# czbiohub-sf/yogo

Measured on AMD Instinct MI355X. Metric: training images/sec (772x1032 gray), higher is better.
Workload: dtype bf16; 1 GPU; BASELINE configs[2]: full train step (fwd+loss+bwd+clamp+AdamW), base_model, 772x1032x1 uint8, 7 classes; per_gpu_batch=128, global_batch=128, parallelism=dp1

## Files before the change

### yogo_amd/csrc/conv_first_fused_bwd.hip

```cpp
#include "common.h"
#include <mutex>
#include <type_traits>
#include <utility>

typedef unsigned int u32x4 __attribute__((ext_vector_type(4)));
typedef int i32x4 __attribute__((ext_vector_type(4)));
typedef float f32x4 __attribute__((ext_vector_type(4)));
typedef float f32x2 __attribute__((ext_vector_type(2)));
typedef __bf16 bf16x8 __attribute__((ext_vector_type(8)));

struct DgFirstParams {
  const u32x4* g;
  const u32x4* wp;
  const unsigned char* img;
  const unsigned short* signs;
  float* part;
  const u32x4* x;
  float* slab;
  float* bias_part;
  int B, H, W, Mpad, act, ncol;
  int tiles_per_row, tile_rows, seg, segs_per_img, nsegs;
  unsigned m_tpr, m_spi;
};

namespace {
constexpr int DF_NJ = 9, DF_PER = 2 * DF_NJ + 2, DF_COUT = 16;
__device__ __forceinline__ int df_udivm1(int n, int d, unsigned m) { return d == 1 ? n : (int)__umulhi((unsigned)n, m); }
__device__ __forceinline__ unsigned df_u(unsigned v) { return (unsigned)__builtin_amdgcn_readfirstlane((int)v); }
__device__ __forceinline__ i32x4 df_rsrc(const void* ptr, unsigned bytes) {
  const unsigned long long a = reinterpret_cast<unsigned long long>(ptr);
  return i32x4{(int)df_u((unsigned)a), (int)df_u((unsigned)(a >> 32) & 0xFFFFu), (int)df_u(bytes), 0x00020000};
}
__device__ __forceinline__ void df_dma16(i32x4 rs, unsigned lds_addr, int voff) {
  unsigned keep;
  lds_addr = df_u(lds_addr);
  asm volatile("s_mov_b32 %0, m0\n\ts_mov_b32 m0, %2\n\ts_nop 4\n\tbuffer_load_dwordx4 %1, %3, 0 offen lds\n\ts_mov_b32 m0, %0"
               : "=&s"(keep) : "v"(voff), "s"(lds_addr), "s"(rs) : "memory");
}
__device__ __forceinline__ void df_dma4(i32x4 rs, unsigned lds_addr, int voff) {
  unsigned keep;
  lds_addr = df_u(lds_addr);
  asm volatile("s_mov_b32 %0, m0\n\ts_mov_b32 m0, %2\n\ts_nop 4\n\tbuffer_load_dword %1, %3, 0 offen lds\n\ts_mov_b32 m0, %0"
               : "=&s"(keep) : "v"(voff), "s"(lds_addr), "s"(rs) : "memory");
}
__device__ __forceinline__ void df_wait_dma() { asm volatile("s_waitcnt vmcnt(0)" ::: "memory"); }
__device__ __forceinline__ bf16x8 df_tr8(const unsigned char* a, int second) {
  typedef __bf16 bf16x4 __attribute__((ext_vector_type(4)));
  typedef bf16x4 __attribute__((address_space(3))) * lds_v4;
  const bf16x4 lo = __builtin_amdgcn_ds_read_tr16_b64_v4bf16((lds_v4)(a));
  const bf16x4 hi = __builtin_amdgcn_ds_read_tr16_b64_v4bf16((lds_v4)(a + second));
  return __builtin_shufflevector(lo, hi, 0, 1, 2, 3, 4, 5, 6, 7);
}
}

#ifndef DF_WAVES_PER_EU
#define DF_WAVES_PER_EU 2
#endif
#ifndef DF_NPF
#define DF_NPF 6
#endif
#ifndef DF_NPF_WG
#define DF_NPF_WG 3
#endif
namespace {
template <class F, int... I>
__device__ __forceinline__ void df_static_for(F&& f, std::integer_sequence<int, I...>) {
  (f(std::integral_constant<int, I>{}), ...);
}
}
template <int R, int NWV, bool WG>
__global__ __launch_bounds__(64 * NWV) __attribute__((amdgpu_waves_per_eu(DF_WAVES_PER_EU))) void conv_bf16_dgrad_first_bwd_kernel(const DgFirstParams p) {
  extern __shared__ __attribute__((aligned(16))) u32x4 lds_u[];
  constexpr int OOB = (int)0x80000000u;
  constexpr int KB = 4, NR = R + 2, ROWU = 34, TU = KB * NR * ROWU, NDMA = (TU + 63) / 64;
  constexpr int IR = 2 * R + 1, IROWB = 72, IDW = IROWB / 4, IU = IR * IDW, NIDMA = (IU + 63) / 64;
  constexpr int SU = R * 16, NSDMA = (SU + 63) / 64;
  static_assert(!WG || (R % 2) == 0, "a piece of the staged x tile is two whole rows");
  constexpr int NXDMA = WG ? R : 0;
  constexpr int WAVE_BYTES = NDMA * 1024 + NIDMA * 256 + NSDMA * 256 + NXDMA * 1024;
  constexpr int CONST_BYTES = ((IR * IROWB + 15) / 16) * 16;
  const int tid = threadIdx.x, lane = tid & 63, c16 = lane & 15, g4 = lane >> 4;
  const int wave = __builtin_amdgcn_readfirstlane(tid >> 6);
  const int H = p.H, W = p.W, IH0 = 2 * H, IW0 = 2 * W;
  const int kcb = H * W * 16;
  const bool leaky = p.act == ACT_LEAKY;
  const unsigned my_addr = (unsigned)(wave * WAVE_BYTES), my_img_addr = my_addr + NDMA * 1024, my_sg_addr = my_img_addr + NIDMA * 256;
  [[maybe_unused]] const unsigned my_x_addr = my_sg_addr + NSDMA * 256;
  const unsigned ones_addr = (unsigned)(NWV * WAVE_BYTES), zeros_addr = ones_addr + CONST_BYTES;
  const u32x4* my_tile = lds_u + wave * (WAVE_BYTES / 16);
  const unsigned char* lds8 = reinterpret_cast<const unsigned char*>(lds_u);
  {
    unsigned* cw = reinterpret_cast<unsigned*>(lds_u) + ones_addr / 4;
    for (int e = tid; e < CONST_BYTES / 4; e += 64 * NWV) {
      cw[e] = 0x01010101u;
      cw[e + CONST_BYTES / 4] = 0u;
    }
  }
  __syncthreads();

  bf16x8 wv[9];
#pragma unroll
  for (int tp = 0; tp < 9; ++tp) wv[tp] = __builtin_bit_cast(bf16x8, p.wp[(tp * KB + g4) * p.Mpad + c16]);

  int rel[NDMA];
  unsigned rc[NDMA];
#pragma unroll
  for (int i = 0; i < NDMA; ++i) {
    const int u = i * 64 + lane;
    const int kb = u / (NR * ROWU), rem = u - kb * (NR * ROWU);
    const int r = rem / ROWU, cc = rem - r * ROWU;
    rel[i] = u < TU ? kb * kcb + (r * W + cc) * 16 : OOB;
    rc[i] = u < TU ? (unsigned)(r << 16 | cc) : 0xFFFFFFFFu;
  }
  unsigned irc[NIDMA];
#pragma unroll
  for (int i = 0; i < NIDMA; ++i) {
    const int e = i * 64 + lane;
    const int r = e / IDW, d = e - r * IDW;
    irc[i] = e < IU ? (unsigned)(r << 16 | d) : 0xFFFFFFFFu;
  }
  const int xj = c16 < 9 ? c16 : 0, kh = xj / 3, kw = xj - 3 * kh;
  const unsigned x_addr = c16 < 9 ? my_img_addr + (unsigned)(kh * IROWB + ((3 + 8 * g4 + kw) & ~3)) : (c16 == 9 ? ones_addr : zeros_addr) + (unsigned)(8 * g4);
  const unsigned x_sh = c16 < 9 ? (unsigned)((3 + kw) & 3) : 0u;
  const unsigned sg_addr = my_sg_addr + (unsigned)(8 * g4);
  const unsigned sg_pos = (unsigned)(c16 < 4 ? c16 : c16 < 8 ? c16 + 4 : c16 < 12 ? c16 - 4 : c16);

  f32x4 d2p = {0.f, 0.f, 0.f, 0.f}, d2n = {0.f, 0.f, 0.f, 0.f};
  f32x4 wacc[WG ? 2 : 1][WG ? 9 : 1], bacc[WG ? 2 : 1];
#pragma unroll
  for (int c = 0; c < (WG ? 2 : 1); ++c) {
    bacc[c] = f32x4{0.f, 0.f, 0.f, 0.f};
#pragma unroll
    for (int t = 0; t < (WG ? 9 : 1); ++t) wacc[c][t] = f32x4{0.f, 0.f, 0.f, 0.f};
  }
  [[maybe_unused]] const unsigned tr_g = my_addr + (unsigned)((((c16 & 3) >> 1) * NR * ROWU + 8 * g4 + (c16 >> 2)) * 16 + (c16 & 1) * 8);
  [[maybe_unused]] const unsigned tr_x = my_x_addr + (unsigned)((((c16 & 3) >> 1) * R * 32 + 8 * g4 + (c16 >> 2)) * 16 + (c16 & 1) * 8);
  const u32x4 ones_op = {0x3F803F80u, 0x3F803F80u, 0x3F803F80u, 0x3F803F80u};

  const int xcd = blockIdx.x & 7, slot = blockIdx.x >> 3, nslot = gridDim.x >> 3;
  const int s8 = (p.nsegs + 7) >> 3, s_end = min(p.nsegs, (xcd + 1) * s8);
  for (int sgm = xcd * s8 + slot * NWV + wave; sgm < s_end; sgm += nslot * NWV) {
    const int b = df_udivm1(sgm, p.segs_per_img, p.m_spi);
    const int t = sgm - b * p.segs_per_img;
    const int sy = df_udivm1(t, p.tiles_per_row, p.m_tpr), ox0 = (t - sy * p.tiles_per_row) * 32;
    const int ty_end = min(p.tile_rows, (sy + 1) * p.seg);
   for (int ty = sy * p.seg; ty < ty_end; ++ty) {
    const int oy0 = ty * R;
    {
      const i32x4 rs_g = df_rsrc(p.g + (size_t)b * KB * H * W, (unsigned)(KB * kcb));
      const int iy0 = oy0 - 1, ix0 = ox0 - 1;
      const int base = (iy0 * W + ix0) * 16;
      if (iy0 >= 0 && iy0 + NR <= H && ix0 >= 0 && ix0 + ROWU <= W) {
#pragma unroll
        for (int i = 0; i < NDMA; ++i) df_dma16(rs_g, my_addr + (unsigned)i * 1024u, (i + 1) * 64 <= TU ? rel[i] + base : (rel[i] == OOB ? OOB : rel[i] + base));
      } else {
#pragma unroll
        for (int i = 0; i < NDMA; ++i) {
          const int r = (int)(rc[i] >> 16), c = (int)(rc[i] & 0xFFFFu);
          const bool ok = ((unsigned)(iy0 + r) < (unsigned)H) && ((unsigned)(ix0 + c) < (unsigned)W);
          df_dma16(rs_g, my_addr + (unsigned)i * 1024u, ok ? rel[i] + base : OOB);
        }
      }
      const i32x4 rs_i = df_rsrc(p.img + (size_t)b * IH0 * IW0, (unsigned)(IH0 * IW0));
      const int jy0 = 2 * oy0 - 1, jx0 = 2 * ox0 - 4;
#pragma unroll
      for (int i = 0; i < NIDMA; ++i) {
        const int r = (int)(irc[i] >> 16), d = (int)(irc[i] & 0xFFFFu);
        const int iy = jy0 + r, ix = jx0 + 4 * d;
        const bool ok = ((unsigned)iy < (unsigned)IH0) && ((unsigned)ix < (unsigned)IW0);
        df_dma4(rs_i, my_img_addr + (unsigned)i * 256u, ok ? iy * IW0 + ix : OOB);
      }
      if (leaky) {
        const i32x4 rs_s = df_rsrc(p.signs + (size_t)b * H * W, (unsigned)(H * W * 2));
#pragma unroll
        for (int i = 0; i < NSDMA; ++i) {
          const int e = i * 64 + lane, r = e >> 4, d = e & 15;
          const bool ok = e < SU && oy0 + r < H && ox0 + 2 * d < W;
          df_dma4(rs_s, my_sg_addr + (unsigned)i * 256u, ok ? ((oy0 + r) * W + ox0 + 2 * d) * 2 : OOB);
        }
      }
      if constexpr (WG) {
        const i32x4 rs_x = df_rsrc(p.x + (size_t)b * 2 * H * W, (unsigned)(2 * kcb));
        const int hi = lane >> 5, col = lane & 31;
        const int xo = ((oy0 + hi) * W + ox0 + col) * 16;
        const bool cok = ox0 + col < W;
#pragma unroll
        for (int i = 0; i < NXDMA; ++i) {
          constexpr int dummy = 0; (void)dummy;
          const int kb = (2 * i) / R, row0 = (2 * i) % R;
          df_dma16(rs_x, my_x_addr + (unsigned)i * 1024u, (cok && oy0 + row0 + hi < H) ? xo + kb * kcb + row0 * W * 16 : OOB);
        }
      }
    }
    const bool right = ox0 + 32 > W;
    df_wait_dma();
    const u32x4* bt = my_tile + g4 * NR * ROWU + c16;
#pragma unroll
    for (int rr = 0; rr < R; ++rr) {
      if (oy0 + rr >= H) break;
      constexpr int NST = WG ? 36 : 18, NPF = WG ? DF_NPF_WG : DF_NPF;
      f32x4 acc[2];
      bf16x8 ring[NPF];
      [[maybe_unused]] bf16x8 xt;
      auto load = [&](auto s_tag) {
        constexpr int S = decltype(s_tag)::value;
        if constexpr (S < 18) {
          constexpr int pb = S / 9, tp = S % 9, ky = tp / 3, kx = tp % 3;
          ring[S % NPF] = __builtin_bit_cast(bf16x8, bt[(rr + ky) * ROWU + 16 * pb + kx]);
        } else {
          constexpr int cbk = (S - 18) / 9, tp = (S - 18) % 9, ky = tp / 3, kx = tp % 3;
          ring[S % NPF] = df_tr8(lds8 + tr_g + ((cbk * 2 * NR + rr + 2 - ky) * ROWU + 2 - kx) * 16, 64);
        }
      };
      auto use = [&](auto s_tag) {
        constexpr int S = decltype(s_tag)::value;
        if constexpr (S < 18) {
          constexpr int pb = S / 9, tp = S % 9;
          acc[pb] = __builtin_amdgcn_mfma_f32_16x16x32_bf16(ring[S % NPF], wv[tp], tp == 0 ? f32x4{0.f, 0.f, 0.f, 0.f} : acc[pb], 0, 0, 0);
        } else if constexpr (WG) {
          constexpr int cbk = (S - 18) / 9, tp = (S - 18) % 9;
          wacc[cbk][tp] = __builtin_amdgcn_mfma_f32_16x16x32_bf16(ring[S % NPF], xt, wacc[cbk][tp], 0, 0, 0);
          if constexpr (tp == 4) bacc[cbk] = __builtin_amdgcn_mfma_f32_16x16x32_bf16(ring[S % NPF], __builtin_bit_cast(bf16x8, ones_op), bacc[cbk], 0, 0, 0);
        }
      };
      unsigned xr[2][3];
      unsigned sw[2][2] = {{0xFFFFFFFFu, 0xFFFFFFFFu}, {0xFFFFFFFFu, 0xFFFFFFFFu}};
      u32x4 xop, gpos, gneg;
      auto p3 = [&](auto k_tag) {
        constexpr int K = decltype(k_tag)::value;
        typedef __bf16 bf16x2 __attribute__((ext_vector_type(2)));
        if constexpr (K == 0) {
#pragma unroll
          for (int pb = 0; pb < 2; ++pb) {
            const unsigned char* xa = lds8 + x_addr + rr * (2 * IROWB) + 32 * pb;
            xr[pb][0] = *reinterpret_cast<const unsigned*>(xa);
            xr[pb][1] = *reinterpret_cast<const unsigned*>(xa + 4);
            xr[pb][2] = *reinterpret_cast<const unsigned*>(xa + 8);
            if (leaky) {
              const unsigned long long s2 = *reinterpret_cast<const unsigned long long*>(lds8 + sg_addr + rr * 64 + 32 * pb);
              sw[pb][0] = (unsigned)s2;
              sw[pb][1] = (unsigned)(s2 >> 32);
            }
          }
        } else if constexpr (K == 1 || K == 2) {
          constexpr int pb = K - 1;
          const unsigned lo4 = __builtin_amdgcn_alignbyte(xr[pb][1], xr[pb][0], x_sh), hi4 = __builtin_amdgcn_alignbyte(xr[pb][2], xr[pb][1], x_sh);
          const unsigned xs = __builtin_amdgcn_perm(hi4, lo4, 0x06040200u);
          const bf16x2 q0 = {(__bf16)(float)(xs & 0xFFu), (__bf16)(float)((xs >> 8) & 0xFFu)};
          const bf16x2 q1 = {(__bf16)(float)((xs >> 16) & 0xFFu), (__bf16)(float)(xs >> 24)};
          xop[2 * pb] = __builtin_bit_cast(unsigned, q0);
          xop[2 * pb + 1] = __builtin_bit_cast(unsigned, q1);
        } else if constexpr (K == 3 || K == 4) {
          constexpr int pb = K - 3;
#pragma unroll
          for (int q = 0; q < 2; ++q) {
            const bf16x2 dq = {(__bf16)acc[pb][2 * q], (__bf16)acc[pb][2 * q + 1]};
            unsigned dw = __builtin_bit_cast(unsigned, dq);
            if (right && ox0 + 16 * pb + 4 * g4 + 2 * q >= W) dw = 0u;
            const unsigned m = leaky ? __umul24((sw[pb][q] >> sg_pos) & 0x00010001u, 0xFFFFu) : 0xFFFFFFFFu;
            const unsigned pos = dw & m;
            gpos[2 * pb + q] = pos;
            gneg[2 * pb + q] = dw ^ pos;
          }
        } else if constexpr (K == 5) {
          d2p = __builtin_amdgcn_mfma_f32_16x16x32_bf16(__builtin_bit_cast(bf16x8, xop), __builtin_bit_cast(bf16x8, gpos), d2p, 0, 0, 0);
        } else {
          d2n = __builtin_amdgcn_mfma_f32_16x16x32_bf16(__builtin_bit_cast(bf16x8, xop), __builtin_bit_cast(bf16x8, gneg), d2n, 0, 0, 0);
        }
      };
      df_static_for([&](auto s_tag) { load(s_tag); }, std::make_integer_sequence<int, NPF>{});
      __builtin_amdgcn_sched_barrier(0);
      df_static_for(
          [&](auto s_tag) {
            constexpr int S = decltype(s_tag)::value;
            use(s_tag);
            if constexpr (S + NPF < NST) load(std::integral_constant<int, S + NPF>{});
            if constexpr (WG) {
              if constexpr (S == 10) xt = df_tr8(lds8 + tr_x + rr * 512, 64);
              if constexpr (S == 18) p3(std::integral_constant<int, 0>{});
              if constexpr (S == 23) p3(std::integral_constant<int, 1>{});
              if constexpr (S == 25) p3(std::integral_constant<int, 2>{});
              if constexpr (S == 27) p3(std::integral_constant<int, 3>{});
              if constexpr (S == 29) p3(std::integral_constant<int, 4>{});
              if constexpr (S == 31) p3(std::integral_constant<int, 5>{});
              if constexpr (S == 32) p3(std::integral_constant<int, 6>{});
            } else {
              if constexpr (S == 12) p3(std::integral_constant<int, 0>{});
              if constexpr (S == 15) p3(std::integral_constant<int, 1>{});
              if constexpr (S == 16) p3(std::integral_constant<int, 2>{});
            }
            __builtin_amdgcn_sched_barrier(0);
          },
          std::make_integer_sequence<int, NST>{});
      if constexpr (!WG) {
        p3(std::integral_constant<int, 3>{});
        p3(std::integral_constant<int, 4>{});
        p3(std::integral_constant<int, 5>{});
        p3(std::integral_constant<int, 6>{});
      }
    }
   }
  }
  float* prow = p.part + (size_t)(blockIdx.x * NWV + wave) * p.ncol;
#pragma unroll
  for (int i = 0; i < 4; ++i) {
    const int j = 4 * g4 + i;
    const float v = d2p[i] + LEAKY_SLOPE * d2n[i];
    if (j < DF_NJ) prow[c16 * DF_PER + j] = v;
    else if (j == DF_NJ) prow[c16 * DF_PER + 2 * DF_NJ] = v;
  }
  if (g4 == 0) prow[c16 * DF_PER + 2 * DF_NJ + 1] = 0.f;
  for (int e = lane; e < DF_COUT * DF_NJ; e += 64) prow[(e / DF_NJ) * DF_PER + DF_NJ + e % DF_NJ] = 0.f;
  for (int e = lane; e < DF_NJ + DF_NJ * DF_NJ; e += 64) prow[DF_COUT * DF_PER + e] = 0.f;
  if constexpr (WG) {
    constexpr int NE = 9 * 32 * 16, STRIDE = NE + 32;
    static_assert(NWV * STRIDE * 4 <= NWV * WAVE_BYTES + 2 * CONST_BYTES, "the reduction uses the kernel's LDS allocation");
    __syncthreads();
    float* red = reinterpret_cast<float*>(lds_u) + wave * STRIDE;
#pragma unroll
    for (int cbk = 0; cbk < 2; ++cbk)
#pragma unroll
      for (int i = 0; i < 4; ++i) {
        const int co = 16 * cbk + 4 * g4 + i;
#pragma unroll
        for (int tp = 0; tp < 9; ++tp) red[(tp * 32 + co) * 16 + c16] = wacc[cbk][tp][i];
        if (c16 == 0) red[NE + co] = bacc[cbk][i];
      }
    __syncthreads();
    const float* r0 = reinterpret_cast<const float*>(lds_u);
    float* sl = p.slab + (size_t)blockIdx.x * NE;
    float* bp = p.bias_part + (size_t)blockIdx.x * 32;
    for (int e = tid; e < STRIDE; e += 64 * NWV) {
      float v = r0[e];
#pragma unroll
      for (int w = 1; w < NWV; ++w) v += r0[w * STRIDE + e];
      if (e < NE) sl[e] = v;
      else bp[e - NE] = v;
    }
  }
}

#ifndef DF_TILE_ROWS
#define DF_TILE_ROWS 6
#endif
#ifndef DF_TILE_ROWS_WG
#define DF_TILE_ROWS_WG 4
#endif
#ifndef DF_WAVES
#define DF_WAVES 4
#endif
namespace {
constexpr int DF_NWV = DF_WAVES;
constexpr int df_rows(bool wg) { return wg ? DF_TILE_ROWS_WG : DF_TILE_ROWS; }
constexpr int df_lds_bytes(int R, int NWV, bool wg) {
  return NWV * (((4 * (R + 2) * 34 + 63) / 64) * 1024 + (((2 * R + 1) * 18 + 63) / 64) * 256 + ((R * 16 + 63) / 64) * 256 + (wg ? R * 1024 : 0)) +
         2 * ((((2 * R + 1) * 72 + 15) / 16) * 16);
}
int df_n_cu() {
  static std::mutex mu;
  static int n_cu_of[64] = {0};
  int dev = 0;
  if (hipGetDevice(&dev) != hipSuccess || dev < 0 || dev >= 64) return -1;
  std::lock_guard<std::mutex> lk(mu);
  if (n_cu_of[dev] == 0) {
    hipDeviceProp_t prop;
    n_cu_of[dev] = (hipGetDeviceProperties(&prop, dev) == hipSuccess && prop.multiProcessorCount > 0) ? prop.multiProcessorCount : 256;
  }
  return n_cu_of[dev];
}
struct DfPlan { int grid, seg; };
DfPlan df_plan(int B, int H, int W, int n_cu, bool wg) {
  const int R = df_rows(wg);
  const int nty = cdiv(H, R), ntx = cdiv(W, 32);
  const int lds = df_lds_bytes(R, DF_NWV, wg);
  const int per_cu = max(1, min(16 / DF_NWV, (160 * 1024) / lds));
#ifdef DF_SEG
  const int seg_lo = DF_SEG, seg_hi = DF_SEG;
#else
  const int seg_lo = 1, seg_hi = 16;
#endif
  DfPlan best{8, 1};
  double best_cost = -1.0;
  for (int seg = seg_lo; seg <= seg_hi && (seg <= nty || seg == seg_lo); ++seg) {
    const long long nsegs = (long long)B * cdiv(nty, seg) * ntx;
    const int s8 = (int)((nsegs + 7) / 8);
    const int grid = 8 * max(1, min(cdiv(s8, DF_NWV), per_cu * n_cu / 8));
    const int waves_per_xcd = grid / 8 * DF_NWV;
    const double cost = (double)cdiv(s8, waves_per_xcd) * min(seg, nty) * (1.0 + (2.0 / R) / min(seg, nty));
    if (best_cost < 0 || cost < best_cost) { best_cost = cost; best = DfPlan{grid, seg}; }
  }
  return best;
}
bool df_shape_ok(int Cmid, int Cout1, int H, int W, int B, int act0, bool wg) {
  if (Cmid != 16 || Cout1 != 32 || H < 1 || W < 2 || (W & 1) || B < 1 || (act0 != ACT_NONE && act0 != ACT_LEAKY)) return false;
  const int R = df_rows(wg);
  if ((long long)4 * H * W * 16 >= (1ll << 31) || (long long)4 * H * W >= (1ll << 31) || (long long)B * cdiv(H, R) * cdiv(W, 32) >= (1ll << 31)) return false;
  const long long tpr = cdiv(W, 32);
  for (int seg = 1; seg <= 16; ++seg) {
    const long long spi = (long long)cdiv(cdiv(H, R), seg) * tpr;
    if (!magic_div_exact((long long)B * spi - 1, (int)spi) || !magic_div_exact(spi, (int)tpr)) return false;
  }
  return true;
}

template <bool WG>
int df_launch(DgFirstParams p, int B, int H, int W, int act0, const char* what, hipStream_t stream) {
  const int n_cu = df_n_cu();
  if (n_cu < 0) {
    yogo_set_error("%s: hipGetDevice failed", what);
    return YOGO_ERR_HIP;
  }
  constexpr int R = df_rows(WG);
  p.B = B; p.H = H; p.W = W; p.Mpad = 32; p.act = act0; p.ncol = DF_COUT * DF_PER + DF_NJ + DF_NJ * DF_NJ;
  const DfPlan pl = df_plan(B, H, W, n_cu, WG);
  p.tiles_per_row = cdiv(W, 32); p.tile_rows = cdiv(H, R); p.seg = pl.seg;
  p.segs_per_img = cdiv(p.tile_rows, pl.seg) * p.tiles_per_row; p.nsegs = B * p.segs_per_img;
  auto magic = [](int d) -> unsigned { return d <= 1 ? 0xFFFFFFFFu : (unsigned)(((1ull << 32) + (unsigned)d - 1ull) / (unsigned)d); };
  p.m_tpr = magic(p.tiles_per_row); p.m_spi = magic(p.segs_per_img);
  const int grid = pl.grid;
  constexpr int lds = df_lds_bytes(R, DF_NWV, WG);
  static_assert(lds <= 160 * 1024, "LDS");
  if (lds > 64 * 1024) {
    static std::mutex mu;
    static bool done[64] = {};
    int dev = 0;
    (void)hipGetDevice(&dev);
    std::lock_guard<std::mutex> lk(mu);
    if (dev >= 0 && dev < 64 && !done[dev]) {
      hipError_t e = hipFuncSetAttribute(reinterpret_cast<const void*>(&conv_bf16_dgrad_first_bwd_kernel<R, DF_NWV, WG>), hipFuncAttributeMaxDynamicSharedMemorySize, lds);
      if (e != hipSuccess) {
        yogo_set_error("%s: hipFuncSetAttribute: %s", what, hipGetErrorString(e));
        return YOGO_ERR_HIP;
      }
      done[dev] = true;
    }
  }
  hipLaunchKernelGGL((conv_bf16_dgrad_first_bwd_kernel<R, DF_NWV, WG>), dim3(grid), dim3(64 * DF_NWV), lds, stream, p);
  if (yogo_launch_log_enabled())
    yogo_launch_log("conv_bf16_dgrad_first_bwd_kernel<%d, %d, %s> | K=32 M=16 at %dx%d segments=%d of %d tiles grid=%d lds=%d act0=%d", R, DF_NWV, WG ? "true" : "false", H, W,
                    p.nsegs, pl.seg, grid, lds, act0);
  hipError_t e = hipGetLastError();
  if (e != hipSuccess) {
    yogo_set_error("%s: launch failed: %s", what, hipGetErrorString(e));
    return YOGO_ERR_HIP;
  }
  return YOGO_OK;
}
}

extern "C" int yogo_internal_wgrad_reduce_q(void* queue, const float* slab, int nslab, int T, int M, int N, int Mpad, int Npad, float clip, float* dw,
                                            const float* bias_part, int nbias, float* db, hipStream_t stream);

extern "C" int yogo_conv2d_dgrad_first_bwd_supported(int Cmid, int Cout1, int H, int W, int B, int act0) {
  return (df_shape_ok(Cmid, Cout1, H, W, B, act0, false) && df_shape_ok(Cmid, Cout1, H, W, B, act0, true)) ? 1 : 0;
}

extern "C" int yogo_conv2d_dgrad_first_bwd_rows(int B, int H, int W, int with_wgrad, int* rows) {
  YOGO_CHECK_ARG(rows && B > 0 && H > 0 && W > 0, "conv2d_dgrad_first_bwd_rows: bad arguments");
  const int n_cu = df_n_cu();
  if (n_cu < 0) {
// ... 48 lines not shown
```

### yogo_amd/csrc/wgrad_bf16.hip

```cpp
#include "common.h"
#include <mutex>
#include <type_traits>
#include <utility>

typedef float f32x16 __attribute__((ext_vector_type(16)));
typedef __bf16 bf16x8 __attribute__((ext_vector_type(8)));
typedef __bf16 bf16x4 __attribute__((ext_vector_type(4)));
typedef unsigned int u32x4 __attribute__((ext_vector_type(4)));

#define WGB_LDS_MAX (160 * 1024)
#ifndef WGB_BLK4
#define WGB_BLK4 1
#endif
#ifndef WGB_BLK4_W
#define WGB_BLK4_W 36
#endif
#define WGB_GSLOTS 4
#define WGB_XSLOTS 6

struct WgradBf16Params {
  const u32x4* x;
  const u32x4* g;
  float* slab;
  float* bias_part;
// ... 164 lines not shown
      }
#define WB_ISSUE_X(i)                                                                                                 \
      if ((i) < p.nxs && (i) * NT + wave * 64 < xtot && !WB_DIAG(4)) {                                                \
        const int c_ = (int)(xrc[i] & 0xFFFFu), r_ = (int)(xrc[i] >> 16);                                             \
        const bool ok_ = ((unsigned)(iy0_ + r_) < (unsigned)p.IH) && ((unsigned)(ix0_ + c_) < (unsigned)p.IW) && (c_ < xneed_) && !WB_DIAG(8) && !(WB_DIAG(32) && r_ >= R); \
        dma16(rs_x, lb_ + (p.xoff + (i) * NT) * 16, ok_ ? xlc[i] + xorg_ : (int)OOB);                                 \
      }
#define WB_ISSUE_SLOTS                                                                                                \
    _Pragma("unroll") for (int i = 0; i < WGB_GSLOTS; ++i) { WB_ISSUE_G(i) }                                          \
    _Pragma("unroll") for (int i = 0; i < WGB_XSLOTS; ++i) { WB_ISSUE_X(i) }
#define WB_ISSUE(BUF)                                                                                                 \
  {                                                                                                                   \
    WB_ISSUE_PREP(BUF)                                                                                                \
    WB_ISSUE_SLOTS                                                                                                    \
  }

  const int gi = lane >> 4, q4 = (lane & 15) >> 2, pc = lane & 3;
  const int lane_ch_off = ((gi & 1) * 16 + pc * 4) * 2;
  const int lane_px = (gi >> 1) * 8 + q4;
  const int ksteps_row = p.wce >> 4;
  const int nsteps = R * ksteps_row;
  const int cnt = (nsteps - ks + KS - 1) / KS;
  const int xpb = p.xcb * 16;
  const int xblk = XR * p.xw * xpb;
  const int gbase = mb * MPW * (R * p.wce * 64) + lane_ch_off;
  const int xbase = p.xoff * 16 + nb * NPW * xblk + (lane_ch_off & (xpb - 1)) + (PACK2 ? (gi & 1) * xpb : 0);
  [[maybe_unused]] const int lean_a0 = BLK4 ? gbase + ((gi >> 1) * 2 * p.wce + q4) * 64 : gbase + lane_px * 64;
  [[maybe_unused]] const int lean_b0 = BLK4 ? xbase + (((gi >> 1) * 2 + tg) * p.xw + q4) * 64 : xbase + ((T == 1 ? 0 : tg) * p.xw + lane_px * WB_SC) * 64;

#define WB_LOAD(AV, BV, I)                                                                                      \
  {                                                                                                             \
    const int st_ = ks + min((I), cnt - 1) * KS;                                                                \
    const int r_ = st_ / ksteps_row;                                                                            \
    const int px_ = (st_ - r_ * ksteps_row) * 16 + lane_px;                                                     \
    const int ga_ = gbase + (r_ * p.wce + px_) * 64;                                                            \
    _Pragma("unroll") for (int m = 0; m < MPW; ++m)                                                             \
      AV[m] = lds_tr8(buf, ga_ + m * (R * p.wce * 64), ga_ + m * (R * p.wce * 64) + 4 * 64);                    \
    _Pragma("unroll") for (int q = 0; q < NPW; ++q)                                                             \
    _Pragma("unroll") for (int t = 0; t < TM; ++t) {                                                            \
      const int xa_ = xbase + q * xblk + (((r_ * S + (T == 1 ? 0 : tg)) * p.xw) + px_ * S + (PACK2 ? 2 * t : t)) * xpb; \
      BV[q][t] = lds_tr8(buf, xa_, xa_ + 4 * S * xpb);                                                          \
    }                                                                                                           \
  }
#define WB_BIAS(AV)                                                                  \
  if (do_bias) {                                                                     \
    _Pragma("unroll") for (int m = 0; m < MPW; ++m)                                  \
    _Pragma("unroll") for (int j = 0; j < 8; ++j) bsum[m] += (float)AV[m][j];        \
  }
#define WB_MFMA(AV, BV)                                           \
  _Pragma("unroll") for (int m = 0; m < MPW; ++m)                 \
  _Pragma("unroll") for (int q = 0; q < NPW; ++q)                 \
  _Pragma("unroll") for (int t = 0; t < TM; ++t)                  \
    acc[m][q][t] = __builtin_amdgcn_mfma_f32_32x32x16_bf16(AV[m], BV[q][t], acc[m][q][t], 0, 0, 0);

  for (int d = 0; d + 1 < p.depth; ++d)
    if (u_begin + d < u_end) WB_ISSUE(d)
  int ib = 0;
  [[maybe_unused]] unsigned long long tw_ = 0, ti_ = 0, tc_ = 0, t0_ = WB_T(), tk_ = t0_;
  constexpr bool LEAN2_OK = KS > 1 && !ROT && (R % KS == 0) && MPW == 1 && NPW == 1;
  auto unit_loop = [&](auto kr_tag, auto mode_tag) {
  [[maybe_unused]] constexpr int KR = decltype(kr_tag)::value;
  [[maybe_unused]] constexpr bool LEAN2 = decltype(mode_tag)::value == 2;
  for (int u = u_begin; u < u_end; ++u) {
    wait_dma(max(0, min(p.depth - 2, u_end - 1 - u)) * my_pieces);
    __builtin_amdgcn_s_barrier();
    asm volatile("" ::: "memory");
    WB_STAMP(tw_)
    const int ahead = p.depth - 1;
    const bool issue_ = u + ahead < u_end;
    int nb_ = ib + ahead;
    nb_ = nb_ >= p.depth ? nb_ - p.depth : nb_;
    if constexpr (!LEAN && !LEAN2) {
      if (issue_) WB_ISSUE(nb_)
    }
    WB_STAMP(ti_)
    const unsigned char* buf = smem_b + ib * p.bufu * 16;
    ib = ib + 1 == p.depth ? 0 : ib + 1;
    if constexpr (BLK4) {
      WB_ISSUE_PREP(nb_)
      const int cwi_ = u % p.nchunk_w;
      constexpr int NSB = KR;
      constexpr int GS = NSB == 8 ? WGB_GSLOTS : 2;
      const bool wide = p.base_w + (cwi_ < p.rem_w ? 1 : 0) > 4 * NSB;
      const int rowa = p.wce * 64, rowx = p.xw * 64;
      const unsigned char* pa0 = buf + lean_a0;
      const unsigned char* pa0j = pa0 + rowa;
      const unsigned char* pa1 = pa0 + R * p.wce * 64;
      const unsigned char* pa1j = pa1 + rowa;
      const unsigned char* pb0 = buf + lean_b0;
      const unsigned char* pb0j = pb0 + rowx;
      typedef bf16x4 __attribute__((address_space(3))) * lds_v4b;
      auto tr2 = [&](const unsigned char* b0, const unsigned char* b1, int off) __attribute__((always_inline)) {
        const bf16x4 lo = __builtin_amdgcn_ds_read_tr16_b64_v4bf16((lds_v4b)(b0 + off));
        const bf16x4 hi = __builtin_amdgcn_ds_read_tr16_b64_v4bf16((lds_v4b)(b1 + off));
        return __builtin_shufflevector(lo, hi, 0, 1, 2, 3, 4, 5, 6, 7);
      };
      bf16x8 av[2][MPW], bvv[2][NPW][TM];
      auto fetch = [&](auto e_tag) __attribute__((always_inline)) {
        constexpr int e = decltype(e_tag)::value, set = e & 1;
        av[set][0] = tr2(pa0, pa0j, e * 256);
#pragma unroll
        for (int t = 0; t < TM; ++t) bvv[set][0][t] = tr2(pb0, pb0j, e * 256 + t * 64);
        if constexpr (MPW == 2) av[set][1] = tr2(pa1, pa1j, e * 256);
      };
      if (!WB_DIAG(2)) {
        fetch(std::integral_constant<int, 0>{});
        auto step = [&](auto e_tag) __attribute__((always_inline)) {
          constexpr int e = decltype(e_tag)::value, set = e & 1;
          if constexpr (e + 1 < NSB) fetch(std::integral_constant<int, e + 1>{});
          else if constexpr (e + 1 == NSB) { if (wide) fetch(std::integral_constant<int, NSB>{}); }
          if (!WB_DIAG(1)) { WB_MFMA(av[set], bvv[set]); }
          if (issue_ && WB_DIAG(64)) {
            if constexpr (e == 0) { WB_ISSUE_SLOTS }
          } else
          if (issue_) {
            if constexpr (e < GS) { WB_ISSUE_G(e) }
            else if constexpr (e < NSB && e - GS < WGB_XSLOTS) { WB_ISSUE_X(e - GS) }
            if constexpr (e == NSB - 1) {
#pragma unroll
              for (int sl = NSB - GS; sl < WGB_XSLOTS; ++sl) { WB_ISSUE_X(sl) }
            }
          }
          if (do_bias) {
            if (--bias_turn < 0) {
              bias_turn = NBW * TG - 1;
#pragma unroll
              for (int m = 0; m < MPW; ++m)
#pragma unroll
                for (int j = 0; j < 8; ++j) bsum[m] += (float)av[set][m][j];
            }
          }
          __builtin_amdgcn_sched_barrier(0);
        };
        wb_static_for(step, std::make_integer_sequence<int, NSB>{});
        if (wide) step(std::integral_constant<int, NSB>{});
      } else if (issue_) {
        WB_ISSUE_SLOTS
      }
    } else
    if constexpr (LEAN) {
      constexpr int KSL = (WGB_GSLOTS + WGB_XSLOTS + R - 1) / R;
      WB_ISSUE_PREP(nb_)
      constexpr int NS = R * KR;
      const unsigned char* pa0 = buf + lean_a0;
      const unsigned char* pa1 = buf + lean_a0 + R * p.wce * 64;
      const unsigned char* pb0 = buf + lean_b0;
      const int rowb = S * p.xw * 64;
      bf16x8 av[2][MPW], bvv[2][NPW][TM];
      auto fetch = [&](auto e_tag) {
        constexpr int e = decltype(e_tag)::value, set = e & 1, r = e / KR, kx = e % KR;
        av[set][0] = lds_tr8(pa0, e * 1024, e * 1024 + 256);
        const unsigned char* pb = pb0 + r * rowb;
#pragma unroll
        for (int q = 0; q < NPW; ++q)
#pragma unroll
          for (int t = 0; t < TM; ++t)
            bvv[set][q][t] = lds_tr8(pb + q * xblk, kx * 1024 * WB_SC + t * 64, kx * 1024 * WB_SC + t * 64 + 256 * WB_SC);
        if constexpr (MPW == 2) av[set][1] = lds_tr8(pa1, e * 1024, e * 1024 + 256);
      };
      if (!WB_DIAG(2)) {
      fetch(std::integral_constant<int, 0>{});
      auto step = [&](auto e_tag) {
        constexpr int e = decltype(e_tag)::value, set = e & 1, r = e / KR, kx = e % KR;
        if constexpr (e + 1 < NS) fetch(std::integral_constant<int, e + 1>{});
        if (!WB_DIAG(1)) { WB_MFMA(av[set], bvv[set]); }
        if (kx == 0 && issue_) {
#pragma unroll
          for (int j = 0; j < KSL; ++j) {
            constexpr int dummy = 0; (void)dummy;
            const int sl = r * KSL + j;
// ... 120 lines not shown
#undef WB_ISSUE_PREP
#undef WB_ISSUE_G
#undef WB_ISSUE_X
#undef WB_LOAD
#undef WB_MFMA
#undef WB_BIAS

  float* sl = p.slab + (size_t)(split * KS + ks) * T * p.Mpad * p.Npad;
  const int m0 = m0b * 8, n0 = n0b * 8;
#pragma unroll
  for (int mi = 0; mi < MPW; ++mi)
#pragma unroll
    for (int q = 0; q < NPW; ++q)
#pragma unroll
      for (int t = 0; t < TM; ++t) {
        const int tap = PACK2 ? 2 * t + (l31 >> 4) : t;
        const int n = n0 + (nb * NPW + q) * 32 + (PACK2 ? (l31 & 15) : l31);
        if (tap < TT) {
#pragma unroll
          for (int r = 0; r < 16; ++r) {
            const int m = m0 + (mb * MPW + mi) * 32 + (r & 3) + 8 * (r >> 2) + 4 * half;
            sl[((size_t)(tg * TT + tap) * p.Mpad + m) * p.Npad + n] = acc[mi][q][t][r];
          }
        }
      }
  if (do_bias) {
    const int brow = LEAN ? (split * KS + ks) * (NBW * TG) + nb * TG + tg : split * KS + ks;
#pragma unroll
    for (int mi = 0; mi < MPW; ++mi) {
      const float tot = bsum[mi] + __shfl_xor(bsum[mi], 32, 64);
      if (half == 0) p.bias_part[(size_t)brow * p.Mpad + m0 + (mb * MPW + mi) * 32 + l31] = tot;
    }
  }
}

extern "C" int yogo_internal_wgrad_reduce_q(void* queue, const float* slab, int nslab, int T, int M, int N, int Mpad, int Npad, float clip, float* dw,
                                            const float* bias_part, int nbias, float* db, hipStream_t stream);
extern "C" int yogo_internal_wgrad_reduce(const float* slab, int nslab, int T, int M, int N, int Mpad, int Npad, float clip, float* dw,
                                          const float* bias_part, int nbias, float* db, hipStream_t stream);

namespace {

thread_local char g_wb_plan_txt[256] = "";

struct WbPlan {
  bool blk4;
  int MBW, NBW, NPW, MPW, KS, R, Mpad, Npad, nchunk_w, base_w, rem_w, wce, nrowg, xw, units, nsplit, units_per_split, ngs, nxs, bufu,
      depth, lds_bytes, xcb, xoff, nsb;
  dim3 grid;
};

bool wb_plan(int B, int N, int M, int IH, int IW, int ks, int stride, WbPlan* pl) {
  const int pad = ks == 3 ? 1 : 0;
  const int OH = (IH + 2 * pad - ks) / stride + 1, OW = (IW + 2 * pad - ks) / stride + 1;
  const int mblocks = cdiv(M, 32), nblocks = cdiv(N, 32);
  int MBW = min(4, mblocks);
  if (MBW == 3) MBW = 2;
  int NBW = min(4 / MBW, nblocks);
  if (NBW == 3) NBW = 2;
  int NPW = (MBW == 4 && NBW == 1 && nblocks >= 2 && ks == 3) ? 2 : 1;
  int MPW = 1;
  if (NPW == 2) { MBW = 2; NBW = 2; NPW = 1; MPW = 2; }
  const int KS = 4 / (MBW * NBW);
  const bool tall = MBW == 1 && NBW == 1 && ks == 3 && stride == 1 && OH >= 64;
  int R = (NPW == 2 || MPW == 2) ? (stride == 1 ? 3 : 2) : (stride == 1 ? (tall ? 8 : 4) : 2);
  bool blk4 = MPW == 2 && stride == 1 && ks == 3 && WGB_BLK4;
  const int R_row = R;
  pl->MBW = MBW; pl->NBW = NBW; pl->NPW = NPW; pl->MPW = MPW; pl->KS = KS;
  pl->Mpad = round_up(M, 32 * MBW * MPW);
  pl->Npad = round_up(N, 32 * NBW * NPW);
  if (blk4) R = 4;
  const int TG = ks == 3 ? 3 : 1;
  const int NT = 64 * MBW * NBW * KS * TG;
  const int XR = ks == 3 ? (R - 1) * stride + 3 : R;
  const int xcb = (NBW * NPW == 1 && N <= 16 && KS != 1) ? 2 : 4;
  pl->xcb = xcb;
  bool found = false;
  int best_waste = 1 << 30;
  pl->depth = 0;
  if (blk4) {
    const int wlist[2] = {WGB_BLK4_W, 36};
    for (int wi = 0; wi < 2 && !found; ++wi) {
      const int w = wlist[wi], xw = w + 2, nsb = w / 4 - 1;
      if (nsb != 8 && nsb != 4) continue;
      const int gtot = MBW * MPW * 4 * R * w, xtot = NBW * NPW * xcb * XR * xw;
      const int ngs = cdiv(gtot, NT), nxs = cdiv(xtot, NT);
      const int xoff = round_up(gtot, 64), bufu = xoff + round_up(xtot, 64);
      if (ngs > (nsb == 8 ? WGB_GSLOTS : 2) || nxs > WGB_XSLOTS || 2 * bufu * 16 > WGB_LDS_MAX) continue;
      int best_steps = 1 << 30, best_nc = 0;
      for (int nc = cdiv(OW, w); nc <= cdiv(OW, w) + 3 && nc <= OW; ++nc) {
        const int base = OW / nc, rem = OW - base * nc;
        if (base + (rem ? 1 : 0) > w) continue;
        const int steps = rem * (base + 1 > 4 * nsb ? nsb + 1 : nsb) + (nc - rem) * (base > 4 * nsb ? nsb + 1 : nsb);
        if (steps < best_steps) { best_steps = steps; best_nc = nc; }
      }
      if (best_nc == 0) continue;
      pl->nchunk_w = best_nc; pl->wce = w; pl->xw = xw; pl->ngs = ngs; pl->nxs = nxs; pl->bufu = bufu; pl->xoff = xoff; pl->nsb = nsb;
      pl->depth = min(4, WGB_LDS_MAX / (bufu * 16));
      found = true;
    }
    if (!found) { blk4 = false; R = R_row; }
  }
  pl->blk4 = blk4;
  pl->R = R;
  const int XR_row = ks == 3 ? (R - 1) * stride + 3 : R;
  for (int wmax = 64; wmax >= 16 && !found; wmax -= 16) {
    for (int nc = cdiv(OW, wmax); nc <= cdiv(OW, wmax) + 4 && nc <= OW; ++nc) {
      const int w = round_up(cdiv(OW, nc), 16);
      if (w > wmax) continue;
      const int xw = (w - 1) * stride + (ks == 3 ? 3 : 1);
      const int ngs = cdiv(MBW * MPW * 4 * R * w, NT), nxs = cdiv(NBW * NPW * xcb * XR_row * xw, NT);
      const int bufu = (ngs + nxs) * NT;
      if (ngs > WGB_GSLOTS || nxs > WGB_XSLOTS || 2 * bufu * 16 > WGB_LDS_MAX) continue;
      const int waste = nc * w - OW;
      if (waste < best_waste) {
        best_waste = waste;
        pl->nchunk_w = nc; pl->wce = w; pl->xw = xw; pl->ngs = ngs; pl->nxs = nxs; pl->bufu = bufu; pl->xoff = ngs * NT; pl->nsb = 0;
        found = true;
      }
    }
  }
  if (!found) return false;
  pl->base_w = OW / pl->nchunk_w;
  pl->rem_w = OW - pl->base_w * pl->nchunk_w;
  if (pl->depth == 0) pl->depth = 3 * pl->bufu * 16 <= WGB_LDS_MAX ? 3 : 2;
  pl->lds_bytes = pl->depth * pl->bufu * 16;
  pl->nrowg = cdiv(OH, R);
  pl->units = B * pl->nrowg * pl->nchunk_w;
  const int gy = pl->Npad / (32 * NBW * NPW), gz = pl->Mpad / (32 * MBW * MPW);
  int nsplit = max(1, min(pl->units, 256 / max(1, gy * gz)));
  pl->units_per_split = cdiv(pl->units, nsplit);
  pl->nsplit = cdiv(pl->units, pl->units_per_split);
  pl->grid = dim3(pl->nsplit, gy, gz);
  return true;
}

int wb_bias_rows(const WbPlan& pl, int T) {
  const bool lean = pl.KS == 1;
  return pl.nsplit * pl.KS * (lean ? pl.NBW * (T == 1 ? 1 : 3) : 1);
}

template <int MBW, int NBW, int NPW, int KS, int T, int S, int R, int MPW = 1, bool ROT = false, bool PACK2 = false, bool BLK4 = false>
int wb_launch_one(const WgradBf16Params& p, const WbPlan& pl, hipStream_t stream) {
  static std::mutex mu;
  static bool done[64] = {false};
  int dev = 0;
  if (hipGetDevice(&dev) != hipSuccess || dev < 0 || dev >= 64) {
    yogo_set_error("wgrad_bf16: hipGetDevice failed");
    return YOGO_ERR_HIP;
  }
  {
    std::lock_guard<std::mutex> lk(mu);
    if (!done[dev]) {
      const hipError_t e = hipFuncSetAttribute(reinterpret_cast<const void*>(&wgrad_bf16_kernel<MBW, NBW, NPW, KS, T, S, R, MPW, ROT, PACK2, BLK4>),
                                               hipFuncAttributeMaxDynamicSharedMemorySize, WGB_LDS_MAX);
      if (e != hipSuccess) {
        yogo_set_error("wgrad_bf16: hipFuncSetAttribute(MaxDynamicSharedMemorySize = %d) failed: %s", WGB_LDS_MAX, hipGetErrorString(e));
        return YOGO_ERR_HIP;
      }
      done[dev] = true;
    }
  }
  hipLaunchKernelGGL((wgrad_bf16_kernel<MBW, NBW, NPW, KS, T, S, R, MPW, ROT, PACK2, BLK4>), pl.grid, dim3(64 * MBW * NBW * KS * (T == 1 ? 1 : 3)),
                     pl.lds_bytes, stream, p);
  yogo_launch_log("wgrad_bf16_kernel<%d, %d, %d, %d, %d, %d, %d, %d, %s, %s, %s> | %s", MBW, NBW, NPW, KS, T, S, R, MPW, ROT ? "true" : "false",
                  PACK2 ? "true" : "false", BLK4 ? "true" : "false", g_wb_plan_txt);
  return YOGO_OK;
// ... 90 lines not shown
```

Before: 11190 images/s.

## Reuse overlapping gradient halo rows via LDS ring in first-layer dgrad

Rearranges the staged gradient tile in the first-layer fused backward kernel into row-pair slots. Consecutive tiles in a segment can then keep the overlapping halo rows and DMA only the new row pairs, with reads alternating between normal and reversed order. This aims to cut redundant global-to-LDS traffic. The wgrad kernel also switches LDS row strides to compile-time constants for the BLK4 path and tightens the planner check so those constants stay valid. The cost is more complex indexing, extra template instantiations for the three staging modes and two read orders, and a risk of LDS bank conflicts from the new layout.

```diff
diff --git a/yogo_amd/csrc/conv_first_fused_bwd.hip b/yogo_amd/csrc/conv_first_fused_bwd.hip
--- a/yogo_amd/csrc/conv_first_fused_bwd.hip
+++ b/yogo_amd/csrc/conv_first_fused_bwd.hip
@@ -62,6 +62,9 @@
 #ifndef DF_NPF_WG
 #define DF_NPF_WG 3
 #endif
+#ifndef DF_RING
+#define DF_RING 1
+#endif
 namespace {
 template <class F, int... I>
 __device__ __forceinline__ void df_static_for(F&& f, std::integer_sequence<int, I...>) {
@@ -72,7 +75,14 @@
 __global__ __launch_bounds__(64 * NWV) __attribute__((amdgpu_waves_per_eu(DF_WAVES_PER_EU))) void conv_bf16_dgrad_first_bwd_kernel(const DgFirstParams p) {
   extern __shared__ __attribute__((aligned(16))) u32x4 lds_u[];
   constexpr int OOB = (int)0x80000000u;
-  constexpr int KB = 4, NR = R + 2, ROWU = 34, TU = KB * NR * ROWU, NDMA = (TU + 63) / 64;
+  constexpr int KB = 4, NR = R + 2, ROWU = 34;
+  static_assert((R % 2) == 0, "the staged gradient rows are kept in pairs");
+  constexpr bool RING = DF_RING != 0;
+  constexpr int HS = RING ? 2 * ROWU : 2 * NR * ROWU, LS = RING ? (2 * HS + 15) / 16 * 16 : NR * ROWU, PU = RING ? 2 * LS : 2 * ROWU;
+  constexpr int NP = NR / 2, TU = RING ? NP * PU : KB * NR * ROWU, NDMA = (TU + 63) / 64;
+  constexpr int TRH = RING ? HS : LS, TRC = RING ? LS : HS;
+  constexpr int NEWU = (NP - 1) * PU, NNEW = (NEWU + 63) / 64;
+  constexpr int PADV = (int)0xC0000000u;
   constexpr int IR = 2 * R + 1, IROWB = 72, IDW = IROWB / 4, IU = IR * IDW, NIDMA = (IU + 63) / 64;
   constexpr int SU = R * 16, NSDMA = (SU + 63) / 64;
   static_assert(!WG || (R % 2) == 0, "a piece of the staged x tile is two whole rows");
@@ -107,10 +117,18 @@
 #pragma unroll
   for (int i = 0; i < NDMA; ++i) {
     const int u = i * 64 + lane;
-    const int kb = u / (NR * ROWU), rem = u - kb * (NR * ROWU);
-    const int r = rem / ROWU, cc = rem - r * ROWU;
-    rel[i] = u < TU ? kb * kcb + (r * W + cc) * 16 : OOB;
-    rc[i] = u < TU ? (unsigned)(r << 16 | cc) : 0xFFFFFFFFu;
+    int kb, r, cc;
+    bool ok;
+    if constexpr (RING) {
+      const int pr = u / PU, rem = u - pr * PU, lo = rem / LS, rem2 = rem - lo * LS, hi = rem2 / HS, rem3 = rem2 - hi * HS;
+      kb = 2 * hi + lo, r = 2 * pr + rem3 / ROWU, cc = rem3 % ROWU;
+      ok = u < TU && rem2 < 2 * HS;
+    } else {
+      kb = u / (NR * ROWU), r = (u - kb * NR * ROWU) / ROWU, cc = u % ROWU;
+      ok = u < TU;
+    }
+    rel[i] = ok ? kb * kcb + (r * W + cc) * 16 : PADV;
+    rc[i] = ok ? (unsigned)(r << 16 | cc) : 0xFFFFFFFFu;
   }
   unsigned irc[NIDMA];
 #pragma unroll
@@ -133,7 +151,7 @@
 #pragma unroll
     for (int t = 0; t < (WG ? 9 : 1); ++t) wacc[c][t] = f32x4{0.f, 0.f, 0.f, 0.f};
   }
-  [[maybe_unused]] const unsigned tr_g = my_addr + (unsigned)((((c16 & 3) >> 1) * NR * ROWU + 8 * g4 + (c16 >> 2)) * 16 + (c16 & 1) * 8);
+  [[maybe_unused]] const unsigned tr_g = my_addr + (unsigned)((((c16 & 3) >> 1) * TRH + 8 * g4 + (c16 >> 2)) * 16 + (c16 & 1) * 8);
   [[maybe_unused]] const unsigned tr_x = my_x_addr + (unsigned)((((c16 & 3) >> 1) * R * 32 + 8 * g4 + (c16 >> 2)) * 16 + (c16 & 1) * 8);
   const u32x4 ones_op = {0x3F803F80u, 0x3F803F80u, 0x3F803F80u, 0x3F803F80u};
 
@@ -146,21 +164,42 @@
     const int ty_end = min(p.tile_rows, (sy + 1) * p.seg);
    for (int ty = sy * p.seg; ty < ty_end; ++ty) {
     const int oy0 = ty * R;
+    const int tk = DF_RING ? ty - sy * p.seg : 0;
+    const int stage_mode = tk == 0 ? 0 : ((tk & 1) ? 1 : 2);
+    const bool rev = (tk & 1) != 0;
     {
       const i32x4 rs_g = df_rsrc(p.g + (size_t)b * KB * H * W, (unsigned)(KB * kcb));
       const int iy0 = oy0 - 1, ix0 = ox0 - 1;
       const int base = (iy0 * W + ix0) * 16;
-      if (iy0 >= 0 && iy0 + NR <= H && ix0 >= 0 && ix0 + ROWU <= W) {
-#pragma unroll
-        for (int i = 0; i < NDMA; ++i) df_dma16(rs_g, my_addr + (unsigned)i * 1024u, (i + 1) * 64 <= TU ? rel[i] + base : (rel[i] == OOB ? OOB : rel[i] + base));
-      } else {
-#pragma unroll
-        for (int i = 0; i < NDMA; ++i) {
-          const int r = (int)(rc[i] >> 16), c = (int)(rc[i] & 0xFFFFu);
-          const bool ok = ((unsigned)(iy0 + r) < (unsigned)H) && ((unsigned)(ix0 + c) < (unsigned)W);
-          df_dma16(rs_g, my_addr + (unsigned)i * 1024u, ok ? rel[i] + base : OOB);
-        }
-      }
+      const bool interior = iy0 >= 0 && iy0 + NR <= H && ix0 >= 0 && ix0 + ROWU <= W;
+      df_static_for(
+          [&](auto m_tag) {
+            constexpr int MODE = decltype(m_tag)::value;
+            if (stage_mode != MODE) return;
+            constexpr int NPC = MODE == 0 ? NDMA : NNEW, RUNU = MODE == 0 ? TU : NEWU;
+            const unsigned dst = my_addr + (MODE == 2 ? (unsigned)(PU * 16) : 0u);
+            df_static_for(
+                [&](auto i_tag) {
+                  constexpr int i = decltype(i_tag)::value;
+                  constexpr int p0 = (64 * i) / PU, cut = (p0 + 1) * PU - 64 * i;
+                  constexpr int dq = MODE == 0 ? 0 : MODE == 2 ? 1 : NP - 1 - 2 * p0, dq2 = MODE == 1 ? dq - 2 : dq;
+                  constexpr bool two = MODE == 1 && cut < 64;
+                  const int tb = RING ? (int)df_u((unsigned)(base + dq * (2 * W * 16))) : base, tb2 = two ? (int)df_u((unsigned)(base + dq2 * (2 * W * 16))) : tb;
+                  int voff = rel[i] + (two ? (lane >= cut ? tb2 : tb) : tb);
+                  if (!interior) {
+                    const int r = (int)(rc[i] >> 16) + 2 * (two ? (lane >= cut ? dq2 : dq) : dq), c = (int)(rc[i] & 0xFFFFu);
+                    const bool ok = ((unsigned)(iy0 + r) < (unsigned)H) && ((unsigned)(ix0 + c) < (unsigned)W);
+                    voff = ok ? voff : OOB;
+                  }
+                  if constexpr (MODE != 0 && (i + 1) * 64 > RUNU) {
+                    if (lane < RUNU - i * 64) df_dma16(rs_g, dst + (unsigned)i * 1024u, voff);
+                  } else {
+                    df_dma16(rs_g, dst + (unsigned)i * 1024u, voff);
+                  }
+                },
+                std::make_integer_sequence<int, NPC>{});
+          },
+          std::make_integer_sequence<int, DF_RING ? 3 : 1>{});
       const i32x4 rs_i = df_rsrc(p.img + (size_t)b * IH0 * IW0, (unsigned)(IH0 * IW0));
       const int jy0 = 2 * oy0 - 1, jx0 = 2 * ox0 - 4;
 #pragma unroll
@@ -194,7 +233,11 @@
     }
     const bool right = ox0 + 32 > W;
     df_wait_dma();
-    const u32x4* bt = my_tile + g4 * NR * ROWU + c16;
+    const u32x4* bt = my_tile + (g4 & 1) * LS + (g4 >> 1) * HS + c16;
+    df_static_for([&](auto rev_tag) __attribute__((always_inline)) {
+    constexpr bool REV = decltype(rev_tag)::value != 0;
+    if (rev != REV) return;
+    auto rowu = [](int r) constexpr { return (REV ? NP - 1 - (r >> 1) : (r >> 1)) * PU + (r & 1) * ROWU; };
 #pragma unroll
     for (int rr = 0; rr < R; ++rr) {
       if (oy0 + rr >= H) break;
@@ -206,10 +249,10 @@
         constexpr int S = decltype(s_tag)::value;
         if constexpr (S < 18) {
           constexpr int pb = S / 9, tp = S % 9, ky = tp / 3, kx = tp % 3;
-          ring[S % NPF] = __builtin_bit_cast(bf16x8, bt[(rr + ky) * ROWU + 16 * pb + kx]);
+          ring[S % NPF] = __builtin_bit_cast(bf16x8, bt[rowu(rr + ky) + 16 * pb + kx]);
         } else {
           constexpr int cbk = (S - 18) / 9, tp = (S - 18) % 9, ky = tp / 3, kx = tp % 3;
-          ring[S % NPF] = df_tr8(lds8 + tr_g + ((cbk * 2 * NR + rr + 2 - ky) * ROWU + 2 - kx) * 16, 64);
+          ring[S % NPF] = df_tr8(lds8 + tr_g + (cbk * TRC + rowu(rr + 2 - ky) + 2 - kx) * 16, 64);
         }
       };
       auto use = [&](auto s_tag) {
@@ -299,6 +342,7 @@
         p3(std::integral_constant<int, 6>{});
       }
     }
+    }, std::make_integer_sequence<int, DF_RING ? 2 : 1>{});
    }
   }
   float* prow = p.part + (size_t)(blockIdx.x * NWV + wave) * p.ncol;
@@ -321,7 +365,7 @@
     for (int cbk = 0; cbk < 2; ++cbk)
 #pragma unroll
       for (int i = 0; i < 4; ++i) {
-        const int co = 16 * cbk + 4 * g4 + i;
+        const int co = DF_RING ? 8 * (cbk + 2 * (g4 >> 1)) + 4 * (g4 & 1) + i : 16 * cbk + 4 * g4 + i;
 #pragma unroll
         for (int tp = 0; tp < 9; ++tp) red[(tp * 32 + co) * 16 + c16] = wacc[cbk][tp][i];
         if (c16 == 0) red[NE + co] = bacc[cbk][i];
@@ -353,7 +397,7 @@
 constexpr int DF_NWV = DF_WAVES;
 constexpr int df_rows(bool wg) { return wg ? DF_TILE_ROWS_WG : DF_TILE_ROWS; }
 constexpr int df_lds_bytes(int R, int NWV, bool wg) {
-  return NWV * (((4 * (R + 2) * 34 + 63) / 64) * 1024 + (((2 * R + 1) * 18 + 63) / 64) * 256 + ((R * 16 + 63) / 64) * 256 + (wg ? R * 1024 : 0)) +
+  return NWV * ((((DF_RING ? (R + 2) / 2 * 288 : 4 * (R + 2) * 34) + 63) / 64) * 1024 + (((2 * R + 1) * 18 + 63) / 64) * 256 + ((R * 16 + 63) / 64) * 256 + (wg ? R * 1024 : 0)) +
          2 * ((((2 * R + 1) * 72 + 15) / 16) * 16);
 }
 int df_n_cu() {
@@ -369,6 +413,14 @@
   return n_cu_of[dev];
 }
 struct DfPlan { int grid, seg; };
+#if defined(YOGO_TEST_HOOKS) || defined(YOGO_DIAG)
+static int g_df_seg = 0;
+extern "C" int yogo_hook_first_bwd_seg(int seg) {
+  YOGO_CHECK_ARG(seg >= 0 && seg <= 16, "yogo_hook_first_bwd_seg: 0 (the planner) or 1 .. 16");
+  g_df_seg = seg;
+  return YOGO_OK;
+}
+#endif
 DfPlan df_plan(int B, int H, int W, int n_cu, bool wg) {
   const int R = df_rows(wg);
   const int nty = cdiv(H, R), ntx = cdiv(W, 32);
@@ -376,6 +428,8 @@
   const int per_cu = max(1, min(16 / DF_NWV, (160 * 1024) / lds));
 #ifdef DF_SEG
   const int seg_lo = DF_SEG, seg_hi = DF_SEG;
+#elif defined(YOGO_TEST_HOOKS) || defined(YOGO_DIAG)
+  const int seg_lo = g_df_seg > 0 ? g_df_seg : 1, seg_hi = g_df_seg > 0 ? g_df_seg : 16;
 #else
   const int seg_lo = 1, seg_hi = 16;
 #endif
diff --git a/yogo_amd/csrc/wgrad_bf16.hip b/yogo_amd/csrc/wgrad_bf16.hip
--- a/yogo_amd/csrc/wgrad_bf16.hip
+++ b/yogo_amd/csrc/wgrad_bf16.hip
@@ -270,10 +270,14 @@
       constexpr int NSB = KR;
       constexpr int GS = NSB == 8 ? WGB_GSLOTS : 2;
       const bool wide = p.base_w + (cwi_ < p.rem_w ? 1 : 0) > 4 * NSB;
-      const int rowa = p.wce * 64, rowx = p.xw * 64;
+#ifdef WGB_RT_STRIDES
+      const int rowa = p.wce * 64, rowx = p.xw * 64, blka = R * p.wce * 64;
+#else
+      constexpr int rowa = 4 * (NSB + 1) * 64, rowx = (4 * (NSB + 1) + 2) * 64, blka = R * rowa;
+#endif
       const unsigned char* pa0 = buf + lean_a0;
       const unsigned char* pa0j = pa0 + rowa;
-      const unsigned char* pa1 = pa0 + R * p.wce * 64;
+      const unsigned char* pa1 = pa0 + blka;
       const unsigned char* pa1j = pa1 + rowa;
       const unsigned char* pb0 = buf + lean_b0;
       const unsigned char* pb0j = pb0 + rowx;
@@ -560,7 +564,7 @@
     const int wlist[2] = {WGB_BLK4_W, 36};
     for (int wi = 0; wi < 2 && !found; ++wi) {
       const int w = wlist[wi], xw = w + 2, nsb = w / 4 - 1;
-      if (nsb != 8 && nsb != 4) continue;
+      if ((nsb != 8 && nsb != 4) || w != 4 * (nsb + 1)) continue;
       const int gtot = MBW * MPW * 4 * R * w, xtot = NBW * NPW * xcb * XR * xw;
       const int ngs = cdiv(gtot, NT), nxs = cdiv(xtot, NT);
       const int xoff = round_up(gtot, 64), bufu = xoff + round_up(xtot, 64);
```

Measured after the change: 11290 images/s (median of 6 runs). About the same (+0.9%).
